# ariana-spalter/human-robot-gym

Measured on AMD Instinct MI355X. Metric: env steps/sec (whole node), ReachHuman+shield 4096 envs, higher is better.
Workload: dtype f64

## Files before the change

human-robot-gym_amd/_lib.py:

```python
import ctypes
import os
import subprocess

from ._cstruct import CONST, EnvState, BoxState, StackState, HammerState, ModelDesc, ClipTable

_HERE = os.path.dirname(os.path.abspath(__file__))
LIB_PATH = os.path.join(_HERE, "libhrgym_hip.so")
_variant = None
SRC = os.path.join(_HERE, "csrc", "hrgym_hip.hip")
SRC_BOX = os.path.join(_HERE, "csrc", "hrgym_box.hip")
SRC_HO = os.path.join(_HERE, "csrc", "hrgym_handover.hip")
SRC_LIFT = os.path.join(_HERE, "csrc", "hrgym_lift.hip")
SRC_STACK = os.path.join(_HERE, "csrc", "hrgym_stack.hip")
SRC_HAMMER = os.path.join(_HERE, "csrc", "hrgym_hammer.hip")
SRC_HULLS = os.path.join(_HERE, "csrc", "hrgym_hulls.hip")
SRC_BOX_HULLS = os.path.join(_HERE, "csrc", "hrgym_box_hulls.hip")

EXPORTS = [
    "hrg_last_error", "hrg_version", "hrg_state_bytes", "hrg_batch_create", "hrg_batch_destroy", "hrg_batch_reset",
    "hrg_batch_step", "hrg_batch_contacts", "hrg_batch_capsules", "hrg_batch_get_state", "hrg_batch_set_state",
    "hrg_batch_kernel_time", "hrg_batch_enable_taps", "hrg_box_bytes", "hrg_batch_get_box", "hrg_batch_set_box", "hrg_batch_get_states", "hrg_batch_set_states",
    "hrg_batch_check_actions", "hrg_stack_bytes", "hrg_batch_get_stack", "hrg_batch_set_stack", "hrg_batch_launch_order",
    "hrg_hammer_bytes", "hrg_batch_get_hammer", "hrg_batch_set_hammer", "hrg_test_hull_queries",
    "hrg_test_hull_box_queries", "hrg_batch_mpr_fallbacks",
]


def build_library(force=False, verbose=False):
    deps = [SRC, SRC_BOX, SRC_HO, SRC_LIFT, SRC_STACK, SRC_HAMMER, SRC_HULLS, SRC_BOX_HULLS] + [os.path.join(_HERE, "csrc", f) for f in ("hrgym_device.h", "hrgym_kernels.h", "hrgym_hull.h")] + [
        os.path.join(os.path.dirname(_HERE), "include", f) for f in ("hrgym.h", "hrgym_state.h")]
    if not force and os.path.exists(LIB_PATH) and all(os.path.getmtime(LIB_PATH) >= os.path.getmtime(d) for d in deps):
        return LIB_PATH
    cmd = ["hipcc", "--offload-arch=gfx950", "-O3", "-std=c++17", "-shared", "-fPIC", "-Wno-unused-value", "-Xarch_device", "-fapprox-func", "-mllvm", "-disable-machine-licm", "-o", LIB_PATH,
           SRC, SRC_BOX, SRC_HO, SRC_LIFT, SRC_STACK, SRC_HAMMER, SRC_HULLS, SRC_BOX_HULLS]
    if verbose:
        print(" ".join(cmd))
    subprocess.check_call(cmd)
    return LIB_PATH


_lib = None


def use_variant_library(path):
    global _variant
    if _lib is not None:
        raise RuntimeError("use_variant_library() must be called before the library is loaded")
    _variant = os.path.abspath(path)


def variant_library():
    return _variant


def load_library():
    global _lib
    if _lib is not None:
# ... 1 lines not shown
    for var in ("HRG_LIB_PATH", "HRG_PHASE_MASK"):
        if os.environ.get(var):
            raise RuntimeError(f"{var} is set: the library no longer honours it (use _lib.use_variant_library() / a -DHRG_STAMPS diagnostic build); unset it")
    path = _variant or LIB_PATH
    if not os.path.exists(path):
        raise RuntimeError(f"{path} is missing: run `python -c 'import __graft_entry__ as g; g.build()'` (hipcc --offload-arch=gfx950). "
                           "There is no CPU fallback for the stepper.")
    lib = ctypes.CDLL(path)
    vp, i32, i64 = ctypes.c_void_p, ctypes.c_int32, ctypes.c_int64
    lib.hrg_last_error.restype = ctypes.c_char_p
    lib.hrg_version.restype = ctypes.c_char_p
    lib.hrg_state_bytes.restype = ctypes.c_size_t
    lib.hrg_batch_create.argtypes = [ctypes.POINTER(ModelDesc), ctypes.POINTER(ClipTable), i32, i64, i32, ctypes.POINTER(vp)]
    lib.hrg_batch_destroy.argtypes = [vp]
    lib.hrg_batch_destroy.restype = None
    lib.hrg_batch_reset.argtypes = [vp, vp, vp, vp]
    lib.hrg_batch_step.argtypes = [vp] * 8
    lib.hrg_batch_contacts.argtypes = [vp, vp, vp]
    lib.hrg_batch_launch_order.argtypes = [vp, vp, vp]
    lib.hrg_batch_capsules.argtypes = [vp, vp, vp, vp]
    lib.hrg_batch_get_state.argtypes = [vp, i32, vp, ctypes.c_size_t]
    lib.hrg_batch_set_state.argtypes = [vp, i32, vp, ctypes.c_size_t]
    lib.hrg_batch_get_states.argtypes = [vp, vp, i32, vp, vp]
    lib.hrg_batch_set_states.argtypes = [vp, vp, i32, vp, vp]
    lib.hrg_box_bytes.restype = ctypes.c_size_t
    lib.hrg_batch_get_box.argtypes = [vp, i32, vp, ctypes.c_size_t]
    lib.hrg_batch_set_box.argtypes = [vp, i32, vp, ctypes.c_size_t]
    lib.hrg_hammer_bytes.restype = ctypes.c_size_t
    lib.hrg_batch_get_hammer.argtypes = [vp, i32, vp, ctypes.c_size_t]
    lib.hrg_batch_set_hammer.argtypes = [vp, i32, vp, ctypes.c_size_t]
    lib.hrg_test_hull_queries.argtypes = [vp, vp, vp, i32, vp]
    lib.hrg_test_hull_box_queries.argtypes = [vp, vp, vp, i32, vp]
    lib.hrg_batch_mpr_fallbacks.argtypes = [vp, ctypes.POINTER(i64)]
    lib.hrg_stack_bytes.restype = ctypes.c_size_t
    lib.hrg_batch_get_stack.argtypes = [vp, i32, vp, ctypes.c_size_t]
    lib.hrg_batch_set_stack.argtypes = [vp, i32, vp, ctypes.c_size_t]
    lib.hrg_batch_enable_taps.argtypes = [vp, i32]
    lib.hrg_batch_check_actions.argtypes = [vp, vp, vp, vp]
    lib.hrg_batch_kernel_time.argtypes = [vp, ctypes.POINTER(ctypes.c_double), ctypes.POINTER(i64)]
    if lib.hrg_state_bytes() != ctypes.sizeof(EnvState):
        raise RuntimeError("hrg_env_state layout mismatch between header mirror and library: rebuild")
    _lib = lib
    return lib


class HrgError(RuntimeError):
    pass


def _check(lib, rc):
    if rc != 0:
        raise HrgError(f"hrgym error {rc}: {lib.hrg_last_error().decode()}")


class HipBatch:

    def __init__(self, desc, clips, n_envs, env_id0=0, device=0, out=None):
        import torch
        if not torch.cuda.is_available():
            raise RuntimeError("HipBatch needs a ROCm GPU (torch.cuda.is_available() is False); there is no CPU fallback")
        self.torch = torch
        self.lib = load_library()
        self.n = int(n_envs)
        self.device = torch.device("cuda", device)
        self._clips = clips
        table = clips.table()
# ... 104 lines not shown
        _check(self.lib, self.lib.hrg_batch_get_hammer(self.h, int(e), ctypes.byref(s), ctypes.sizeof(s)))
        return s

    def set_hammer(self, e, s):
        _check(self.lib, self.lib.hrg_batch_set_hammer(self.h, int(e), ctypes.byref(s), ctypes.sizeof(s)))

    def get_stack(self, e):
        s = StackState()
        _check(self.lib, self.lib.hrg_batch_get_stack(self.h, int(e), ctypes.byref(s), ctypes.sizeof(s)))
        return s

    def set_stack(self, e, s):
        _check(self.lib, self.lib.hrg_batch_set_stack(self.h, int(e), ctypes.byref(s), ctypes.sizeof(s)))

    def contacts(self):
        import numpy as np
        pairs = np.zeros((self.n, CONST["HRG_NCON_MAX"], 2), np.int32)
        ncon = np.zeros(self.n, np.int32)
        _check(self.lib, self.lib.hrg_batch_contacts(self.h, pairs.ctypes.data_as(ctypes.c_void_p), ncon.ctypes.data_as(ctypes.c_void_p)))
        return pairs, ncon

    def launch_order(self):
        import numpy as np
        order = np.zeros(self.n, np.int32)
        nb = ctypes.c_int32(0)
        _check(self.lib, self.lib.hrg_batch_launch_order(self.h, order.ctypes.data_as(ctypes.c_void_p), ctypes.byref(nb)))
        return order, int(nb.value)

    def mpr_fallbacks(self):
        c = ctypes.c_int64()
        _check(self.lib, self.lib.hrg_batch_mpr_fallbacks(self.h, ctypes.byref(c)))
        return c.value

    def enable_taps(self, on=True):
        _check(self.lib, self.lib.hrg_batch_enable_taps(self.h, int(bool(on))))

    def capsules(self):
        import numpy as np
        r = np.zeros((self.n, CONST["HRG_NSHIELD_RCAP"], 7))
        h = np.zeros((self.n, CONST["HRG_NHCAP_MAX"], 7))
        nh = np.zeros(self.n, np.int32)
        vp = ctypes.c_void_p
        _check(self.lib, self.lib.hrg_batch_capsules(self.h, r.ctypes.data_as(vp), h.ctypes.data_as(vp), nh.ctypes.data_as(vp)))
        return r, h, nh

    def kernel_time(self):
        ms, n = ctypes.c_double(), ctypes.c_int64()
        _check(self.lib, self.lib.hrg_batch_kernel_time(self.h, ctypes.byref(ms), ctypes.byref(n)))
        return ms.value, n.value

    def close(self):
        if getattr(self, "h", None) and self.h.value:
            self.lib.hrg_batch_destroy(self.h)
            self.h = ctypes.c_void_p()

    def __del__(self):
        try:
            self.close()
        except Exception:
            pass
```

human-robot-gym_amd/csrc/hrgym_device.h:

```cpp
#pragma once
#include <hip/hip_runtime.h>
#include <stdint.h>

#include "../../include/hrgym.h"
#include "../../include/hrgym_state.h"

#define NV HRG_NV
#define NARM HRG_NARM
#ifndef HRG_BOX
#define HRG_BOX 0
#endif
#ifndef HRG_LIFT
#define HRG_LIFT 0
#endif
#ifndef HRG_HANDOVER
#define HRG_HANDOVER 0
#endif
#ifndef HRG_STACK
#define HRG_STACK 0
#endif
#ifndef HRG_HULLS
#define HRG_HULLS 0
#endif
#ifndef HRG_HAMMER
#define HRG_HAMMER 0
#endif
#define HRG_BASE_TU (!HRG_BOX && !HRG_STACK && !HRG_HAMMER && !HRG_HULLS)
#define NVT HRG_NVT
#if HRG_HAMMER
#define NVS HRG_NV_HAMMER
#define NCON_DYN HRG_NCON_DYN_HAMMER
#define HM_OB NV
#define HM_ON (NV + 6)
#define HM_OH (NV + 8)
#elif HRG_STACK
#define NVS HRG_NV_STACK
#define NCON_DYN HRG_NCON_DYN_STACK
#define NCUBE HRG_NCUBE
#elif HRG_BOX
#define NVS NVT
#define NCON_DYN HRG_NCON_DYN_BOX
#else
#define NVS NV
#define NCON_DYN HRG_NCON_DYN
#endif
#define BODY_BOX 100
#define DI __device__ __forceinline__
#ifndef HRG_MIN_WAVES
#define HRG_MIN_WAVES 4
#endif
#ifndef HRG_PHASE
#define HRG_PHASE __device__ __forceinline__
#endif
#define PH_DYNTERMS HRG_PHASE
#define PH_HUMAN HRG_PHASE
#define PH_SHIELD HRG_PHASE
#define PH_COLLIDE HRG_PHASE
#define PH_CLASSIFY HRG_PHASE
#define PH_DYNSTEP HRG_PHASE
#define HRG_PI 3.14159265358979323846
// ... 20 lines not shown
#define STAMP_FLUSH(lane)
#define COUNT(k, n) do { if (threadIdx.x == 0) g_acc[k] += (n); } while (0)
#define STAMP_FINAL(lane) do { __syncthreads(); if ((lane) < 32) atomicAdd(&g_stamps[lane], g_acc[lane]); { unsigned long long _te; STAMP_NOW(_te); if (_te - g_tbeg > g_slow_thresh) { if ((lane) < 32) atomicAdd(&g_stamps_slow[lane], g_acc[lane]); if ((lane) == 32) atomicAdd(&g_stamps_slow[32], 1ull); if ((lane) == 33) atomicAdd(&g_stamps_slow[33], _te - g_tbeg); } } if ((lane) < 32 && blockIdx.x < 16384) g_envacc[blockIdx.x][lane] = g_acc[lane]; if ((lane) == 0 && blockIdx.x < 16384) { unsigned long long _t; STAMP_NOW(_t); g_envcyc[blockIdx.x][0] = g_tbeg; g_envcyc[blockIdx.x][1] = _t; unsigned _hw, _xcc; asm volatile("s_getreg_b32 %0, hwreg(HW_REG_HW_ID)\n\ts_getreg_b32 %1, hwreg(HW_REG_XCC_ID)" : "=s"(_hw), "=s"(_xcc)); g_envcyc[blockIdx.x][2] = ((unsigned long long)_xcc << 32) | _hw; } } while (0)
#else
#define STAMP_DECL
#define STAMP_INIT(lane)
#define STAMP(k)
#define STAMP_FLUSH(lane)
#define COUNT(k, n)
#define STAMP_FINAL(lane)
#endif

struct DevModel {
  hrg_model_desc m;
  double Rbase[9];
  double Rq[NV][9];
  int32_t anc_mask[NV];
  int32_t hb_maxdepth;
  double sol_K, sol_Bd;
  double rcap_hl[HRG_NRCAP], hcap_hl[HRG_NHB];
  int32_t hb_njump;
  int32_t hb_jump[4][HRG_NHB];
  int32_t phase_mask;
  hrg_path brake_full;
  double brake_T, brake_ds;
  int32_t hc_n;
  int32_t hc_kind[HRG_NHCAP_MAX], hc_j1[HRG_NHCAP_MAX], hc_j2[HRG_NHCAP_MAX];
  double hc_th[HRG_NHCAP_MAX], hc_v[HRG_NHCAP_MAX], hc_a[HRG_NHCAP_MAX], hc_len[HRG_NHCAP_MAX];
  int32_t n_self;
  int32_t self_i[64], self_j[64];
  int32_t n_chk;
  int32_t chk_i[32], chk_j[32];
  hrg_clip_table clips;
  const double* hull_dev;
  double hull_cen[HRG_NHULL][3];
  unsigned long long* mpr_fallback;
};

static inline void hull_centroids(const double* verts, const int32_t* off, double cen[HRG_NHULL][3]) {
  for (int h = 0; h < HRG_NHULL; h++) {
    double s[3] = {0, 0, 0};
    for (int i = off[h]; i < off[h + 1]; i++) for (int a = 0; a < 3; a++) s[a] += verts[3 * i + a];
    for (int a = 0; a < 3; a++) cen[h][a] = s[a] / (double)(off[h + 1] - off[h]);
  }
}

struct Contact {
  int32_t g1, g2, b1, b2;
  double dist, n[3], pos[3];
};

#define ROW_CON0 24
#define ROW_WELD0 (ROW_CON0 + 4 * NCON_DYN)
#if HRG_HAMMER
#define HROW_NFRIC 8
#define HROW_LIM0 9
#define HROW_NLIM 25
#define HROW_EQ0 27
#define HROW_CON0 36
#define HROW_NEQ 9
#define NROW 128
#elif HRG_STACK
#define SROW_WELD0 24
#define SROW_CON0 36
#define NROW HRG_NROW_STACK
#elif HRG_BOX && (HRG_HANDOVER || HRG_LIFT)
// ... 730 lines not shown
```

human-robot-gym_amd/csrc/hrgym_hip.hip:

```cpp
#include <hip/hip_runtime.h>

#include <cmath>
#include <cstdio>
#include <cstring>
#include <cstdlib>
#include <memory>
#include <string>
#include <vector>

#include "hrgym_kernels.h"

template <class MD>
DI void impedance(const MD& m, double x0, double* imp) {
  const double d0 = m.solimp[0], dmax = m.solimp[1], width = m.solimp[2], mid = m.solimp[3], power = m.solimp[4];
  const double x = fabs(x0) / width;
  double y;
  if (x >= 1) y = 1;
  else if (x <= 0) y = 0;
  else if (x <= mid) { const double u = x / mid; y = u * u * mid; }
  else { const double u = (1 - x) / (1 - mid); y = 1 - u * u * (1 - mid); }
  (void)power;
  *imp = d0 + y * (dmax - d0);
}

// ... 2820 lines not shown
  const double* src = (const double*)(states + e);
  double* dst = (double*)&L.st;
  constexpr int NW = (int)(sizeof(hrg_env_state) / sizeof(double));
  for (int k = lane; k < NW; k += 64) dst[k] = src[k];
  wave_sync();
  env_reset(dm, lane, env_id0 + e, obs ? obs + (size_t)e * HRG_OBS_DIM : nullptr);
  wave_sync();
  hrg_env_state* st_out = states;
  asm volatile("" : "+s"(st_out));
  double* out = (double*)(st_out + e);
  for (int k = lane; k < NW; k += 64) out[k] = dst[k];
#if HRG_BOX || HRG_STACK || HRG_HAMMER
  box_store(boxes, e, lane);
#endif
}

#if HRG_BASE_TU
__global__ __launch_bounds__(64 * HRG_WG_WAVES, HRG_KERNEL_WAVES) void hrg_check_kernel(const DevModel* __restrict__ dm_, const hrg_env_state* __restrict__ states, const double* __restrict__ actions,
                                                                          uint8_t* __restrict__ collides, int n_envs) {
  const int e = hrg_env(), lane = hrg_lane();
  if (e >= n_envs) return;
  Lds& L = g_L;
  const double* src = (const double*)(states + e);
  double* dst = (double*)&L.st;
  constexpr int NW = (int)(sizeof(hrg_env_state) / sizeof(double));
  for (int k = lane; k < NW; k += 64) dst[k] = src[k];
  if (lane < NV) L.act[lane] = lane < HRG_ACT_DIM ? actions[(size_t)e * HRG_ACT_DIM + lane] : 0.0;
  wave_sync();
  const ModelPtr dm = uniform_model(dm_);
  action_goal(dm, lane, L.act);
  const bool hit = config_collides(dm_, lane);
  if (lane == 0) collides[e] = hit ? 1 : 0;
}
#endif

extern "C" __attribute__((visibility("hidden"))) void hrg_box_launch_step(int n_envs, hipStream_t st, const DevModel* dm, hrg_env_state* states, double* actions, float* obs, float* term_obs,
                                                                           float* reward, uint8_t* done, int32_t* info, double* dbg_r, double* dbg_h, int32_t* dbg_nh, int64_t env_id0,
                                                                           float* scratch_obs, hrg_box_state* boxes, StepOrder ord);
extern "C" __attribute__((visibility("hidden"))) void hrg_box_launch_reset(int n_envs, hipStream_t st, const DevModel* dm, hrg_env_state* states, const uint8_t* mask, float* obs,
                                                                            int64_t env_id0, hrg_box_state* boxes);
#if HRG_BASE_TU
extern "C" __attribute__((visibility("hidden"))) void hrg_stack_launch_step(int n_envs, hipStream_t st, const DevModel* dm, hrg_env_state* states, double* actions, float* obs, float* term_obs,
                                                                             float* reward, uint8_t* done, int32_t* info, double* dbg_r, double* dbg_h, int32_t* dbg_nh, int64_t env_id0,
                                                                             float* scratch_obs, hrg_stack_state* stacks, StepOrder ord);
extern "C" __attribute__((visibility("hidden"))) void hrg_stack_launch_reset(int n_envs, hipStream_t st, const DevModel* dm, hrg_env_state* states, const uint8_t* mask, float* obs,
                                                                              int64_t env_id0, hrg_stack_state* stacks);
#endif
#if HRG_BASE_TU
extern "C" __attribute__((visibility("hidden"))) void hrg_hammer_launch_step(int n_envs, hipStream_t st, const DevModel* dm, hrg_env_state* states, double* actions, float* obs, float* term_obs,
                                                                              float* reward, uint8_t* done, int32_t* info, double* dbg_r, double* dbg_h, int32_t* dbg_nh, int64_t env_id0,
                                                                              float* scratch_obs, hrg_hammer_state* hammers, StepOrder ord);
extern "C" __attribute__((visibility("hidden"))) void hrg_hammer_launch_reset(int n_envs, hipStream_t st, const DevModel* dm, hrg_env_state* states, const uint8_t* mask, float* obs,
                                                                               int64_t env_id0, hrg_hammer_state* hammers);
extern "C" __attribute__((visibility("hidden"))) void hrg_ho_launch_step(int n_envs, hipStream_t st, const DevModel* dm, hrg_env_state* states, double* actions, float* obs, float* term_obs,
                                                                          float* reward, uint8_t* done, int32_t* info, double* dbg_r, double* dbg_h, int32_t* dbg_nh, int64_t env_id0,
                                                                          float* scratch_obs, hrg_box_state* boxes, StepOrder ord);
extern "C" __attribute__((visibility("hidden"))) void hrg_ho_launch_reset(int n_envs, hipStream_t st, const DevModel* dm, hrg_env_state* states, const uint8_t* mask, float* obs,
                                                                           int64_t env_id0, hrg_box_state* boxes);
extern "C" __attribute__((visibility("hidden"))) void hrg_lift_launch_step(int n_envs, hipStream_t st, const DevModel* dm, hrg_env_state* states, double* actions, float* obs, float* term_obs,
                                                                            float* reward, uint8_t* done, int32_t* info, double* dbg_r, double* dbg_h, int32_t* dbg_nh, int64_t env_id0,
                                                                            float* scratch_obs, hrg_box_state* boxes, StepOrder ord);
extern "C" __attribute__((visibility("hidden"))) void hrg_lift_launch_reset(int n_envs, hipStream_t st, const DevModel* dm, hrg_env_state* states, const uint8_t* mask, float* obs,
                                                                             int64_t env_id0, hrg_box_state* boxes);
#endif
#if HRG_BASE_TU
extern "C" __attribute__((visibility("hidden"))) void hrg_box_hull_launch_step(int n_envs, hipStream_t st, const DevModel* dm, hrg_env_state* states, double* actions, float* obs, float* term_obs,
// ... 91 lines not shown
#define hrg_debug_envcyc hrg_debug_envcyc_ho
#elif HRG_LIFT
#define hrg_debug_envacc hrg_debug_envacc_lift
#define hrg_debug_envcyc hrg_debug_envcyc_lift
#elif HRG_BOX
#define hrg_debug_envacc hrg_debug_envacc_box
#define hrg_debug_envcyc hrg_debug_envcyc_box
#elif HRG_HULLS
#define hrg_debug_envacc hrg_debug_envacc_hull
#define hrg_debug_envcyc hrg_debug_envcyc_hull
#endif
#if 1
extern "C" int hrg_debug_envacc(unsigned long long* out, int n) { return hipMemcpyFromSymbol(out, HIP_SYMBOL(g_envacc), sizeof(unsigned long long) * 32 * n) == hipSuccess ? 0 : -1; }
extern "C" int hrg_debug_envcyc(unsigned long long* out, int n) { return hipMemcpyFromSymbol(out, HIP_SYMBOL(g_envcyc), sizeof(unsigned long long) * 3 * n) == hipSuccess ? 0 : -1; }
#endif
#endif

#if HRG_BASE_TU

static thread_local std::string g_err;
static int fail(int code, const std::string& msg) { g_err = msg; return code; }
#define HIPCHK(x)                                                                                         \
  do {                                                                                                    \
    hipError_t _e = (x);                                                                                  \
    if (_e != hipSuccess) return fail(HRG_ERR_HIP, std::string(#x) + ": " + hipGetErrorString(_e));        \
  } while (0)

struct hrg_batch {
  int device = 0;
  int32_t n_envs = 0;
  int64_t env_id0 = 0;
  DevModel* d_model = nullptr;
  double* d_frames = nullptr;
  double* d_hull = nullptr;
  bool hulls = false;
  unsigned long long* d_mpr_fallback = nullptr;
  hrg_env_state* d_states = nullptr;
  double* d_rcaps = nullptr;
  double* d_hcaps = nullptr;
  int32_t* d_nh = nullptr;
  float* d_scratch_obs = nullptr;
  hrg_box_state* d_boxes = nullptr;
  hrg_stack_state* d_stacks = nullptr;
  hrg_hammer_state* d_hammers = nullptr;
  int32_t* d_order = nullptr;
  int32_t parity = 0;
  int32_t task = HRG_TASK_REACH;
  bool timing = false;
  bool taps = false;
  std::vector<std::pair<hipEvent_t, hipEvent_t>> events;
  std::vector<std::pair<hipEvent_t, hipEvent_t>> pool;
};

static int32_t* fair_table(int device) {
  static int32_t* tab[64] = {nullptr};
  if (device < 0 || device >= 64) return nullptr;
  if (!tab[device]) {
    int32_t* p = nullptr;
    if (hipMalloc(&p, sizeof(int32_t) * HRG_FAIR_SLOTS) != hipSuccess) return nullptr;
    if (hipMemset(p, 0, sizeof(int32_t) * HRG_FAIR_SLOTS) != hipSuccess) { hipFree(p); return nullptr; }
    tab[device] = p;
  }
  return tab[device];
}

static void mat_from_quat(double* M, const double* q) {
  double w = q[0], x = q[1], y = q[2], z = q[3];
  M[0] = 1 - 2 * (y * y + z * z); M[1] = 2 * (x * y - w * z); M[2] = 2 * (x * z + w * y);
  M[3] = 2 * (x * y + w * z); M[4] = 1 - 2 * (x * x + z * z); M[5] = 2 * (y * z - w * x);
  M[6] = 2 * (x * z - w * y); M[7] = 2 * (y * z + w * x); M[8] = 1 - 2 * (x * x + y * y);
}

extern "C" {

const char* hrg_last_error(void) { return g_err.c_str(); }
const char* hrg_version(void) { return "hrgym-hip 0.1.0 (gfx950)"; }
size_t hrg_state_bytes(void) { return sizeof(hrg_env_state); }
size_t hrg_box_bytes(void) { return sizeof(hrg_box_state); }
size_t hrg_stack_bytes(void) { return sizeof(hrg_stack_state); }
size_t hrg_hammer_bytes(void) { return sizeof(hrg_hammer_state); }

int hrg_batch_create(const hrg_model_desc* desc, const hrg_clip_table* clips, int32_t n_envs, int64_t env_id0, int32_t device, hrg_batch** out) {
  if (!desc || !clips || !out || n_envs <= 0) return fail(HRG_ERR_INVALID, "null argument or n_envs <= 0");
  if (desc->failsafe_sdot != 0.0) return fail(HRG_ERR_INVALID, "failsafe_sdot must be 0: SSM / OFF brake to a stop, PFL computes its speed from pfl_v_safe / pfl_reach");
  if (desc->shield_type == HRG_SHIELD_PFL) {
    if (!(desc->pfl_v_safe > 0)) return fail(HRG_ERR_INVALID, "PFL: pfl_v_safe must be positive");
    for (int j = 0; j < NARM; j++) if (!(desc->pfl_reach[j] > 0)) return fail(HRG_ERR_INVALID, "PFL: pfl_reach must be positive");
  }
  for (int i = 0; i < NARM; i++)
    if (!(desc->jnt_damping[i] >= 0 && desc->timestep * desc->jnt_damping[i] * desc->dof_invweight0[i] < 1e-3))
      return fail(HRG_ERR_UNSUPPORTED, "arm joint damping too large for the implicit-damping expansion (h d / M must stay below 1e-3; robot.xml: 1e-4)");
  if ((desc->jnt_damping[NARM] > 0) != (desc->jnt_damping[NARM + 1] > 0)) return fail(HRG_ERR_UNSUPPORTED, "the two finger slides must both carry damping, or neither");
  if (desc->solimp[4] != 2.0) return fail(HRG_ERR_UNSUPPORTED, "solimp power must be 2 (MuJoCo's default): the HIP stepper evaluates the impedance sigmoid as a square");
  if (clips->n_clips < 1 || clips->n_clips > HRG_MAX_CLIPS || clips->n_clips != desc->n_clips) return fail(HRG_ERR_INVALID, "clip table / desc.n_clips mismatch");
  for (int i = 0; i < NV; i++) {
    if ((i < NARM) != (desc->jnt_type[i] == 0)) return fail(HRG_ERR_INVALID, "expected 6 hinges followed by 2 slides");
    if (i < NARM && desc->body_parent[i] != i - 1) return fail(HRG_ERR_INVALID, "arm must be a serial chain");
// ... 96 lines not shown
  hm->hc_n = n;
  int ns = 0;
  for (int i = 0; i < HRG_NRCAP; i++)
    for (int j = i + 1; j < HRG_NRCAP; j++)
      if ((desc->rcap_selfmask[i] >> j) & 1u) { hm->self_i[ns] = i; hm->self_j[ns] = j; ns++; }
  hm->n_self = ns;
  int nc = 0;
  for (int i = 0; i < 8; i++)
    for (int j = i + 1; j < 8; j++)
      if (((desc->chk_selfmask[i] >> j) & 1u) && nc < 32) { hm->chk_i[nc] = i; hm->chk_j[nc] = j; nc++; }
  hm->n_chk = nc;
  hm->phase_mask = 0xff;
  {
    double se, ve, ae;
    path_plan(&hm->brake_full, 0.0, 1.0, 0.0, desc->failsafe_sdot, desc->path_amax, desc->path_jmax);
    hm->brake_T = path_total(&hm->brake_full);
    path_eval(&hm->brake_full, hm->brake_T, desc->failsafe_sdot, &se, &ve, &ae);
    hm->brake_ds = se;
  }
#ifdef HRG_STAMPS
  if (const char* pm = getenv("HRG_PHASE_MASK")) hm->phase_mask = atoi(pm);
#endif
  const size_t fbytes = sizeof(double) * HRG_FRAME_DIM * (size_t)clips->total_frames;
  int64_t tot = 0;
  for (int c = 0; c < clips->n_clips; c++) {
    if (clips->clip_len[c] < 1 || clips->clip_offset[c] != tot) { return bail(HRG_ERR_INVALID, "clip table must be densely packed"); }
    tot += clips->clip_len[c];
  }
  if (tot != clips->total_frames) { return bail(HRG_ERR_INVALID, "clip table total_frames mismatch"); }
  HIPCHK_C(hipMalloc(&b->d_frames, fbytes));
  HIPCHK_C(hipMemcpy(b->d_frames, clips->frames, fbytes, hipMemcpyHostToDevice));
  hm->clips = *clips;
  hm->clips.frames = b->d_frames;
  hm->hull_dev = nullptr;
  if (desc->robot_hulls) {
    if (!(desc->task == HRG_TASK_REACH || desc->task == HRG_TASK_PICK_PLACE || desc->task == HRG_TASK_INSPECTION || desc->task == HRG_TASK_POINTING || desc->task == HRG_TASK_REACH_BOX))
      return bail(HRG_ERR_UNSUPPORTED, "robot_hulls: the hull variants of the step kernel exist for ReachHuman and the cube tasks (PickPlace, Inspection, ReachHuman with reach_box)");
    b->hulls = true;
    if (!desc->hull_verts || desc->hull_off[0] != 0) return bail(HRG_ERR_INVALID, "robot_hulls: hull_verts / hull_off missing");
    for (int h = 0; h < HRG_NHULL; h++)
      if (!(desc->hull_off[h + 1] > desc->hull_off[h] + 3 && desc->hull_off[h + 1] <= 1000000)) return bail(HRG_ERR_INVALID, "robot_hulls: every hull needs at least four vertices");
    const size_t hbytes = sizeof(double) * 3 * (size_t)desc->hull_off[HRG_NHULL];
    HIPCHK_C(hipMalloc(&b->d_hull, hbytes));
    HIPCHK_C(hipMemcpy(b->d_hull, desc->hull_verts, hbytes, hipMemcpyHostToDevice));
    hm->hull_dev = b->d_hull;
    hull_centroids(desc->hull_verts, desc->hull_off, hm->hull_cen);
    HIPCHK_C(hipMalloc(&b->d_mpr_fallback, sizeof(unsigned long long)));
    HIPCHK_C(hipMemset(b->d_mpr_fallback, 0, sizeof(unsigned long long)));
    hm->mpr_fallback = b->d_mpr_fallback;
  }
  HIPCHK_C(hipMalloc(&b->d_model, sizeof(DevModel)));
  HIPCHK_C(hipMemcpy(b->d_model, hm, sizeof(DevModel), hipMemcpyHostToDevice));
  HIPCHK_C(hipMalloc(&b->d_states, sizeof(hrg_env_state) * (size_t)n_envs));
  std::vector<hrg_env_state> init((size_t)n_envs);
  memset(init.data(), 0, sizeof(hrg_env_state) * (size_t)n_envs);
  for (auto& s : init) s.episode = -1;
  HIPCHK_C(hipMemcpy(b->d_states, init.data(), sizeof(hrg_env_state) * (size_t)n_envs, hipMemcpyHostToDevice));
  HIPCHK_C(hipMalloc(&b->d_rcaps, sizeof(double) * 7 * HRG_NSHIELD_RCAP * (size_t)n_envs));
  HIPCHK_C(hipMalloc(&b->d_hcaps, sizeof(double) * 7 * HRG_NHCAP_MAX * (size_t)n_envs));
  HIPCHK_C(hipMalloc(&b->d_nh, sizeof(int32_t) * (size_t)n_envs));
  HIPCHK_C(hipMalloc(&b->d_scratch_obs, sizeof(float) * HRG_OBS_DIM * (size_t)n_envs));
  HIPCHK_C(hipMemset(b->d_rcaps, 0, sizeof(double) * 7 * HRG_NSHIELD_RCAP * (size_t)n_envs));
  HIPCHK_C(hipMemset(b->d_hcaps, 0, sizeof(double) * 7 * HRG_NHCAP_MAX * (size_t)n_envs));
  HIPCHK_C(hipMemset(b->d_nh, 0, sizeof(int32_t) * (size_t)n_envs));
  HIPCHK_C(hipMalloc(&b->d_boxes, sizeof(hrg_box_state) * (size_t)n_envs));
  HIPCHK_C(hipMemset(b->d_boxes, 0, sizeof(hrg_box_state) * (size_t)n_envs));
  if (desc->task == HRG_TASK_HAMMERING) {
    HIPCHK_C(hipMalloc(&b->d_hammers, sizeof(hrg_hammer_state) * (size_t)n_envs));
    HIPCHK_C(hipMemset(b->d_hammers, 0, sizeof(hrg_hammer_state) * (size_t)n_envs));
  }
  if (desc->task == HRG_TASK_STACKING) {
    HIPCHK_C(hipMalloc(&b->d_stacks, sizeof(hrg_stack_state) * (size_t)n_envs));
    HIPCHK_C(hipMemset(b->d_stacks, 0, sizeof(hrg_stack_state) * (size_t)n_envs));
  }
  {
    std::vector<int32_t> ord(2 * (size_t)n_envs + 4, 0);
    for (int32_t e = 0; e < n_envs; e++) ord[e] = ord[(size_t)n_envs + e] = e;
    HIPCHK_C(hipMalloc(&b->d_order, sizeof(int32_t) * ord.size()));
    HIPCHK_C(hipMemcpy(b->d_order, ord.data(), sizeof(int32_t) * ord.size(), hipMemcpyHostToDevice));
  }
#undef HIPCHK_C
  *out = b;
  return HRG_OK;
}

void hrg_batch_destroy(hrg_batch* b) {
  if (!b) return;
  hipSetDevice(b->device);
  hipDeviceSynchronize();
  for (auto& p : b->events) { hipEventDestroy(p.first); hipEventDestroy(p.second); }
  for (auto& p : b->pool) { hipEventDestroy(p.first); hipEventDestroy(p.second); }
  hipFree(b->d_model); hipFree(b->d_frames); hipFree(b->d_hull); hipFree(b->d_mpr_fallback); hipFree(b->d_states); hipFree(b->d_rcaps); hipFree(b->d_hcaps); hipFree(b->d_nh); hipFree(b->d_scratch_obs); hipFree(b->d_boxes); hipFree(b->d_stacks); hipFree(b->d_hammers); hipFree(b->d_order);
  delete b;
}

int hrg_batch_reset(hrg_batch* b, const uint8_t* mask_dev, float* obs_dev, void* stream) {
  if (!b) return fail(HRG_ERR_INVALID, "null batch");
  HIPCHK(hipSetDevice(b->device));
  if (b->task == HRG_TASK_HAMMERING) hrg_hammer_launch_reset(b->n_envs, (hipStream_t)stream, b->d_model, b->d_states, mask_dev, obs_dev, b->env_id0, b->d_hammers);
  else if (b->task == HRG_TASK_STACKING) hrg_stack_launch_reset(b->n_envs, (hipStream_t)stream, b->d_model, b->d_states, mask_dev, obs_dev, b->env_id0, b->d_stacks);
  else if (b->task == HRG_TASK_LIFTING) hrg_lift_launch_reset(b->n_envs, (hipStream_t)stream, b->d_model, b->d_states, mask_dev, obs_dev, b->env_id0, b->d_boxes);
  else if (HRG_IS_HANDOVER(b->task)) hrg_ho_launch_reset(b->n_envs, (hipStream_t)stream, b->d_model, b->d_states, mask_dev, obs_dev, b->env_id0, b->d_boxes);
  else if (b->task != HRG_TASK_REACH && b->hulls) hrg_box_hull_launch_reset(b->n_envs, (hipStream_t)stream, b->d_model, b->d_states, mask_dev, obs_dev, b->env_id0, b->d_boxes);
  else if (b->task != HRG_TASK_REACH) hrg_box_launch_reset(b->n_envs, (hipStream_t)stream, b->d_model, b->d_states, mask_dev, obs_dev, b->env_id0, b->d_boxes);
  else if (b->hulls) hrg_hull_launch_reset(b->n_envs, (hipStream_t)stream, b->d_model, b->d_states, mask_dev, obs_dev, b->env_id0);
  else hipLaunchKernelGGL(hrg_reset_kernel, HRG_LAUNCH_DIMS(b->n_envs), 0, (hipStream_t)stream, b->d_model, b->d_states, mask_dev, obs_dev, b->env_id0, b->d_boxes, b->n_envs);
  HIPCHK(hipGetLastError());
  return HRG_OK;
}

int hrg_batch_check_actions(hrg_batch* b, const double* actions_dev, uint8_t* collides_dev, void* stream) {
  if (!b || !actions_dev || !collides_dev) return fail(HRG_ERR_INVALID, "null argument");
  HIPCHK(hipSetDevice(b->device));
  hipLaunchKernelGGL(hrg_check_kernel, HRG_LAUNCH_DIMS(b->n_envs), 0, (hipStream_t)stream, b->d_model, b->d_states, actions_dev, collides_dev, b->n_envs);
  HIPCHK(hipGetLastError());
  return HRG_OK;
}

int hrg_batch_step(hrg_batch* b, double* actions_dev, float* obs_dev, float* term_obs_dev, float* reward_dev, uint8_t* done_dev, int32_t* info_dev, void* stream) {
  if (!b || !actions_dev || !obs_dev || !reward_dev || !done_dev || !info_dev) return fail(HRG_ERR_INVALID, "null argument");
  HIPCHK(hipSetDevice(b->device));
  hipStream_t st = (hipStream_t)stream;
  std::pair<hipEvent_t, hipEvent_t> ev;
  if (b->timing) {
    if (!b->pool.empty()) { ev = b->pool.back(); b->pool.pop_back(); }
    else { HIPCHK(hipEventCreate(&ev.first)); HIPCHK(hipEventCreate(&ev.second)); }
// ... 205 lines not shown
```

human-robot-gym_amd/csrc/hrgym_kernels.h:

```cpp
#pragma once
#include "hrgym_device.h"
#if HRG_HULLS
#include "hrgym_hull.h"
#endif

DI void robot_chain_fk(const DevModel* __restrict__ dm_, int lane, bool shield_on) {
  const ModelPtr dm = uniform_model(dm_);
  Lds& L = g_L;
  double* sc = &L.rc[0][0];
  if (lane < 3 * NARM && (lane >= 2 * NARM || shield_on)) {
    const int cfg = lane / NARM, i = lane - NARM * cfg;
    const double q = cfg == 0 ? L.cq[i] : (cfg == 1 ? L.qe[i] : L.st.qpos[i]);
    double sn, cs;
    sincos_small(q, &sn, &cs);
    sc[2 * lane] = sn; sc[2 * lane + 1] = cs;
  }
  wave_sync();
  if (lane < 9 && (lane >= 6 || shield_on)) {
    const auto& m = dm->m;
    const int cfg = lane / 3, row = lane - 3 * cfg;
    double r0 = dm->Rbase[3 * row], r1 = dm->Rbase[3 * row + 1], r2 = dm->Rbase[3 * row + 2];
    double p = m.base_pos[row];
#pragma unroll 1
    for (int i = 0; i < NARM; i++) {
// ... 239 lines not shown
      const int hd = lane == bl ? 0 : 1;
      const double sn = hd == 0 ? -1.0 : 1.0;
      double Rm[9], q[4], site[3], t[3];
      for (int a = 0; a < 3; a++) { Rm[3 * a] = -sn * R[3 * a + 2]; Rm[3 * a + 1] = R[3 * a + 1]; Rm[3 * a + 2] = sn * R[3 * a]; }
      const double tr = Rm[0] + Rm[4] + Rm[8];
      if (tr > 0) { const double S = fsqrt(tr + 1.0) * 2; q[0] = 0.25 * S; q[1] = (Rm[7] - Rm[5]) / S; q[2] = (Rm[2] - Rm[6]) / S; q[3] = (Rm[3] - Rm[1]) / S; }
      else if (Rm[0] > Rm[4] && Rm[0] > Rm[8]) { const double S = fsqrt(1.0 + Rm[0] - Rm[4] - Rm[8]) * 2; q[0] = (Rm[7] - Rm[5]) / S; q[1] = 0.25 * S; q[2] = (Rm[1] + Rm[3]) / S; q[3] = (Rm[2] + Rm[6]) / S; }
      else if (Rm[4] > Rm[8]) { const double S = fsqrt(1.0 + Rm[4] - Rm[0] - Rm[8]) * 2; q[0] = (Rm[2] - Rm[6]) / S; q[1] = (Rm[1] + Rm[3]) / S; q[2] = 0.25 * S; q[3] = (Rm[5] + Rm[7]) / S; }
      else { const double S = fsqrt(1.0 + Rm[8] - Rm[0] - Rm[4]) * 2; q[0] = (Rm[3] - Rm[1]) / S; q[1] = (Rm[2] + Rm[6]) / S; q[2] = (Rm[5] + Rm[7]) / S; q[3] = 0.25 * S; }
      m3mulv(t, R, m.hb_anchor[b]);
      v3add(site, p, t);
      for (int a = 0; a < 4; a++) L.hm.mocap_quat[hd][a] = q[a];
      for (int a = 0; a < 3; a++) L.hm.mocap_pos[hd][a] = site[a];
    }
  }
#endif
  {
    const int k = lane < HRG_NHJ ? lane : 0;
    const int sb = m.meas_body[k];
    double Rs[9], ps[3];
#pragma unroll
    for (int a = 0; a < 9; a++) Rs[a] = __shfl(R[a], sb, 64);
#pragma unroll
    for (int a = 0; a < 3; a++) ps[a] = __shfl(p[a], sb, 64);
    if (lane < HRG_NHJ) {
      double t[3];
      m3mulv(t, Rs, m.hb_anchor[sb]);
      v3add(L.st.human_site[k], ps, t);
    }
  }
  wave_sync();
}

DI void human_pose_fk(const DevModel* __restrict__ dm_, int lane, int clip, int at, int hold_body = -1, int hold_left = 0) {
  const ModelPtr dm = uniform_model(dm_);
  Lds& L = g_L;
  const auto& m = dm->m;
  hrg_env_state& s = L.st;
  const double* fr = dm->clips.frames + (dm->clips.clip_offset[clip] + at) * HRG_FRAME_DIM;
  double qi[4] = {dm->clips.clip_quat[clip][3], dm->clips.clip_quat[clip][0], dm->clips.clip_quat[clip][1], dm->clips.clip_quat[clip][2]};
  double qbi[4], Rbi[9], pa[3], pr[3], mp[3], mq[4], q1[4];
  quatmul(qbi, m.human_base_quat, qi);
  quat2mat(Rbi, qbi);
  for (int a = 0; a < 3; a++) pa[a] = fr[a] + dm->clips.clip_pos_offset[clip][a];
  m3mulv(pr, Rbi, pa);
  v3add(mp, pr, s.human_pos_offset);
  double qa[4] = {fr[6], fr[3], fr[4], fr[5]};
  quatmul(q1, s.human_rot_offset, qbi);
  quatmul(mq, q1, qa);
  human_fk_lanes(dm_, lane, mp, mq, fr + 7, hold_body, hold_left);
}

#if HRG_BOX || HRG_STACK || HRG_HAMMER
DI double loop_prop(ModelPtr dm, int64_t gid, int episode, int ai, int clip, int k, int speed) {
  double base = speed ? dm->clips.clip_loop_speed[clip][k % HRG_MAX_LOOP] : dm->clips.clip_loop_amp[clip][k % HRG_MAX_LOOP];
  if (k >= HRG_MAX_LOOP) base = speed ? dm->clips.clip_loop2_speed[clip][k - HRG_MAX_LOOP] : dm->clips.clip_loop2_amp[clip][k - HRG_MAX_LOOP];
  const double sf = speed ? dm->clips.clip_loop_speed_std[clip] : dm->clips.clip_loop_amp_std[clip];
  const double z = clampd(rng_gauss(dm->m.seed, (uint64_t)gid, (uint64_t)episode, STREAM_LOOP, (uint64_t)((ai * 2 * HRG_MAX_LOOP + k) * 2 + speed)), -3.0, 3.0);
  return base * exp(z * log(sf));
}
DI double layered_sines(ModelPtr dm, int64_t gid, int episode, int ai, int clip, int kfirst, int n, double t, double start) {
  static_assert(2 * HRG_MAX_LOOP <= 64, "one lane per loop property");
  const int lane = hrg_lane(), kk = lane % HRG_MAX_LOOP, sp = (lane / HRG_MAX_LOOP) & 1;
  const double mine = loop_prop(dm, gid, episode, ai, clip, kfirst + (kk < n ? kk : 0), sp);
  double sum = 0;
  for (int k = 0; k < n; k++) {
    const double A = __shfl(mine, k), S = __shfl(mine, HRG_MAX_LOOP + k);
    sum += A * sin((t - start) / (A / S)) + start;
  }
  return sum - start * (double)(n - 1);
}
#endif

PH_HUMAN void human_control(const DevModel* __restrict__ dm_, int lane, int64_t gid) {
  const ModelPtr dm = uniform_model(dm_);
  Lds& L = g_L;
  const auto& m = dm->m;
  hrg_env_state& s = L.st;
  int control_time = (int)floor((double)s.low_level_time / m.anim_step_length);
  int at = control_time - s.anim_start_time;
  int anim_index = s.anim_index, anim_start = s.anim_start_time;
  int clip = clip_of(dm, gid, s.episode, anim_index);
#if HRG_BOX
// ... 1194 lines not shown
```

include/hrgym.h:

```cpp
#ifndef HRGYM_H
#define HRGYM_H

#include <stddef.h>
#include <stdint.h>

#ifdef __cplusplus
extern "C" {
#endif

#define HRG_NARM 6
#define HRG_NFINGER 2
#define HRG_NV (HRG_NARM + HRG_NFINGER)
#define HRG_NHB 24
#define HRG_NHJ 23
#define HRG_NHQ 69
#define HRG_NRCAP 10
#define HRG_NHULL 7
#define HRG_NSHIELD_RCAP 7
#define HRG_NBODYPART_MAX 20
#define HRG_NEXTREMITY_MAX 4
#define HRG_NHCAP_MAX 64
#define HRG_LTT_NSEG 12
#define HRG_OBS_DIM 64
#define HRG_ACT_DIM 7
// ... 250 lines not shown
const char* hrg_version(void);

size_t hrg_state_bytes(void);

int hrg_batch_create(const hrg_model_desc* desc, const hrg_clip_table* clips, int32_t n_envs,
                     int64_t env_id0, int32_t device, hrg_batch** out);
void hrg_batch_destroy(hrg_batch* b);

int hrg_batch_reset(hrg_batch* b, const uint8_t* mask_dev, float* obs_dev, void* stream);

int hrg_batch_step(hrg_batch* b, double* actions_dev, float* obs_dev, float* term_obs_dev,
                   float* reward_dev, uint8_t* done_dev, int32_t* info_dev, void* stream);

int hrg_batch_contacts(hrg_batch* b, int32_t* pairs_host, int32_t* ncon_host);
int hrg_batch_capsules(hrg_batch* b, double* robot_host, double* human_host, int32_t* n_human_host);
int hrg_batch_launch_order(hrg_batch* b, int32_t* order_host, int32_t* n_busy_host);
int hrg_batch_enable_taps(hrg_batch* b, int32_t on);
int hrg_batch_get_state(hrg_batch* b, int32_t env, void* buf_host, size_t bytes);
int hrg_batch_set_state(hrg_batch* b, int32_t env, const void* buf_host, size_t bytes);
int hrg_batch_get_states(hrg_batch* b, const int32_t* envs_host, int32_t n, void* states_host, void* boxes_host);
int hrg_batch_set_states(hrg_batch* b, const int32_t* envs_host, int32_t n, const void* states_host, const void* boxes_host);
size_t hrg_box_bytes(void);
int hrg_batch_get_box(hrg_batch* b, int32_t env, void* buf_host, size_t bytes);
int hrg_batch_set_box(hrg_batch* b, int32_t env, const void* buf_host, size_t bytes);
size_t hrg_stack_bytes(void);
int hrg_batch_get_stack(hrg_batch* b, int32_t env, void* buf_host, size_t bytes);
int hrg_batch_set_stack(hrg_batch* b, int32_t env, const void* buf_host, size_t bytes);
size_t hrg_hammer_bytes(void);
int hrg_batch_get_hammer(hrg_batch* b, int32_t env, void* buf_host, size_t bytes);
int hrg_batch_set_hammer(hrg_batch* b, int32_t env, const void* buf_host, size_t bytes);
int hrg_test_hull_queries(const double* verts_host, const int32_t* off_host, const void* queries_host, int32_t n, double* out_host);
int hrg_test_hull_box_queries(const double* verts_host, const int32_t* off_host, const void* queries_host, int32_t n, double* out_host);
int hrg_batch_mpr_fallbacks(hrg_batch* b, int64_t* count_host);

int hrg_batch_check_actions(hrg_batch* b, const double* actions_dev, uint8_t* collides_dev, void* hip_stream);

int hrg_batch_kernel_time(hrg_batch* b, double* avg_ms, int64_t* n_launches);

#ifdef __cplusplus
}
#endif
#endif
```

Before: 4.076 million.

## Precompute per-frame human pose table at batch creation for reach and lift

At batch creation, a kernel runs the human forward kinematics once for every clip frame in a root-relative frame and stores the capsule endpoints, joint sites and root position in a device table. During stepping, reach and lift tasks then rebuild the human pose with one rotation plus translation per lane from the table, replacing the per-step tree FK. The cost is extra device memory and an init-time kernel. Hold-body handling is dropped on this path, and a debug comparison kernel is added to check the table against live FK.

Result: faster. 4.500 million, median of 6 (+10.4%).

```diff
diff --git a/human-robot-gym_amd/_lib.py b/human-robot-gym_amd/_lib.py
--- a/human-robot-gym_amd/_lib.py
+++ b/human-robot-gym_amd/_lib.py
@@ -22,7 +22,7 @@
     "hrg_batch_kernel_time", "hrg_batch_enable_taps", "hrg_box_bytes", "hrg_batch_get_box", "hrg_batch_set_box", "hrg_batch_get_states", "hrg_batch_set_states",
     "hrg_batch_check_actions", "hrg_stack_bytes", "hrg_batch_get_stack", "hrg_batch_set_stack", "hrg_batch_launch_order",
     "hrg_hammer_bytes", "hrg_batch_get_hammer", "hrg_batch_set_hammer", "hrg_test_hull_queries",
-    "hrg_test_hull_box_queries", "hrg_batch_mpr_fallbacks",
+    "hrg_test_hull_box_queries", "hrg_batch_mpr_fallbacks", "hrg_batch_pose_table_bytes", "hrg_debug_pose_compare",
 ]
 
 
@@ -90,6 +90,8 @@
     lib.hrg_test_hull_queries.argtypes = [vp, vp, vp, i32, vp]
     lib.hrg_test_hull_box_queries.argtypes = [vp, vp, vp, i32, vp]
     lib.hrg_batch_mpr_fallbacks.argtypes = [vp, ctypes.POINTER(i64)]
+    lib.hrg_batch_pose_table_bytes.argtypes = [vp, ctypes.POINTER(i64)]
+    lib.hrg_debug_pose_compare.argtypes = [vp, vp, i32, vp]
     lib.hrg_stack_bytes.restype = ctypes.c_size_t
     lib.hrg_batch_get_stack.argtypes = [vp, i32, vp, ctypes.c_size_t]
     lib.hrg_batch_set_stack.argtypes = [vp, i32, vp, ctypes.c_size_t]
@@ -260,6 +262,11 @@
         _check(self.lib, self.lib.hrg_batch_mpr_fallbacks(self.h, ctypes.byref(c)))
         return c.value
 
+    def pose_table_bytes(self):
+        c = ctypes.c_int64()
+        _check(self.lib, self.lib.hrg_batch_pose_table_bytes(self.h, ctypes.byref(c)))
+        return c.value
+
     def enable_taps(self, on=True):
         _check(self.lib, self.lib.hrg_batch_enable_taps(self.h, int(bool(on))))
 
diff --git a/human-robot-gym_amd/csrc/hrgym_device.h b/human-robot-gym_amd/csrc/hrgym_device.h
--- a/human-robot-gym_amd/csrc/hrgym_device.h
+++ b/human-robot-gym_amd/csrc/hrgym_device.h
@@ -26,6 +26,11 @@
 #define HRG_HAMMER 0
 #endif
 #define HRG_BASE_TU (!HRG_BOX && !HRG_STACK && !HRG_HAMMER && !HRG_HULLS)
+#define HRG_POSE_TABLE ((!HRG_BOX && !HRG_STACK && !HRG_HAMMER) || HRG_LIFT)
+#define HRG_POSE_HCAP 0
+#define HRG_POSE_SITE (6 * HRG_NHB)
+#define HRG_POSE_ROOT (HRG_POSE_SITE + 3 * HRG_NHJ)
+#define HRG_POSE_DIM (HRG_POSE_ROOT + 3)
 #define NVT HRG_NVT
 #if HRG_HAMMER
 #define NVS HRG_NV_HAMMER
@@ -112,6 +117,7 @@
   int32_t n_chk;
   int32_t chk_i[32], chk_j[32];
   hrg_clip_table clips;
+  const double* pose_tab;
   const double* hull_dev;
   double hull_cen[HRG_NHULL][3];
   unsigned long long* mpr_fallback;
diff --git a/human-robot-gym_amd/csrc/hrgym_hip.hip b/human-robot-gym_amd/csrc/hrgym_hip.hip
--- a/human-robot-gym_amd/csrc/hrgym_hip.hip
+++ b/human-robot-gym_amd/csrc/hrgym_hip.hip
@@ -2876,6 +2876,56 @@
   const bool hit = config_collides(dm_, lane);
   if (lane == 0) collides[e] = hit ? 1 : 0;
 }
+
+__global__ __launch_bounds__(64) void hrg_pose_table_kernel(const DevModel* __restrict__ dm_, double* __restrict__ tab) {
+  const ModelPtr dm = uniform_model(dm_);
+  const int lane = hrg_lane();
+  const int64_t f = (int64_t)blockIdx.x;
+  if (f >= dm->clips.total_frames) return;
+  Lds& L = g_L;
+  int clip = 0;
+  for (int c = 1; c < dm->clips.n_clips; c++)
+    if (f >= dm->clips.clip_offset[c]) clip = c;
+  const double* fr = dm->clips.frames + f * HRG_FRAME_DIM;
+  double qbi[4], qa[4], c[3], mq[4];
+  human_root(dm, clip, fr, c, qbi, qa);
+  quatmul(mq, qbi, qa);
+  const double p0[3] = {0, 0, 0};
+  human_fk_lanes(dm_, lane, p0, mq, fr + 7);
+  double* e = tab + f * HRG_POSE_DIM;
+  for (int k = lane; k < 6 * HRG_NHB; k += 64) e[HRG_POSE_HCAP + k] = (&L.hcap[0][0])[k];
+  for (int k = lane; k < 3 * HRG_NHJ; k += 64) e[HRG_POSE_SITE + k] = (&L.st.human_site[0][0])[k];
+  if (lane < 3) e[HRG_POSE_ROOT + lane] = c[lane];
+}
+
+struct PoseQuery { double pos_off[3], rot_off[4]; int32_t clip, at; };
+__global__ __launch_bounds__(64) void hrg_pose_compare_kernel(const DevModel* __restrict__ dm_, const PoseQuery* __restrict__ q, int n, double* __restrict__ out) {
+  const ModelPtr dm = uniform_model(dm_);
+  const int lane = hrg_lane(), k = (int)blockIdx.x;
+  if (k >= n) return;
+  Lds& L = g_L;
+  hrg_env_state& s = L.st;
+  if (lane < 3) s.human_pos_offset[lane] = q[k].pos_off[lane];
+  if (lane < 4) s.human_rot_offset[lane] = q[k].rot_off[lane];
+  wave_sync();
+  const int clip = __builtin_amdgcn_readfirstlane(q[k].clip), at = __builtin_amdgcn_readfirstlane(q[k].at);
+  const int64_t f = dm->clips.clip_offset[clip] + at;
+  const double* fr = dm->clips.frames + f * HRG_FRAME_DIM;
+  double qbi[4], qa[4], c[3], mp[3], mq[4], q1[4];
+  human_root(dm, clip, fr, c, qbi, qa);
+  v3add(mp, c, s.human_pos_offset);
+  quatmul(q1, s.human_rot_offset, qbi);
+  quatmul(mq, q1, qa);
+  human_fk_lanes(dm_, lane, mp, mq, fr + 7);
+  constexpr int NP = 6 * HRG_NHB + 3 * HRG_NHJ;
+  double* o = out + (size_t)k * 2 * NP;
+  for (int j = lane; j < 6 * HRG_NHB; j += 64) o[j] = (&L.hcap[0][0])[j];
+  for (int j = lane; j < 3 * HRG_NHJ; j += 64) o[6 * HRG_NHB + j] = (&s.human_site[0][0])[j];
+  wave_sync();
+  human_pose_from_table(dm, lane, f);
+  for (int j = lane; j < 6 * HRG_NHB; j += 64) o[NP + j] = (&L.hcap[0][0])[j];
+  for (int j = lane; j < 3 * HRG_NHJ; j += 64) o[NP + 6 * HRG_NHB + j] = (&s.human_site[0][0])[j];
+}
 #endif
 
 extern "C" __attribute__((visibility("hidden"))) void hrg_box_launch_step(int n_envs, hipStream_t st, const DevModel* dm, hrg_env_state* states, double* actions, float* obs, float* term_obs,
@@ -3033,6 +3083,8 @@
   int64_t env_id0 = 0;
   DevModel* d_model = nullptr;
   double* d_frames = nullptr;
+  double* d_pose = nullptr;
+  size_t pose_bytes = 0;
   double* d_hull = nullptr;
   bool hulls = false;
   unsigned long long* d_mpr_fallback = nullptr;
@@ -3064,6 +3116,8 @@
   }
   return tab[device];
 }
+
+static bool hrg_task_uses_pose_table(int task) { return task == HRG_TASK_REACH || task == HRG_TASK_LIFTING; }
 
 static void mat_from_quat(double* M, const double* q) {
   double w = q[0], x = q[1], y = q[2], z = q[3];
@@ -3226,6 +3280,12 @@
   HIPCHK_C(hipMemcpy(b->d_frames, clips->frames, fbytes, hipMemcpyHostToDevice));
   hm->clips = *clips;
   hm->clips.frames = b->d_frames;
+  hm->pose_tab = nullptr;
+  if (hrg_task_uses_pose_table(desc->task)) {
+    b->pose_bytes = sizeof(double) * HRG_POSE_DIM * (size_t)clips->total_frames;
+    HIPCHK_C(hipMalloc(&b->d_pose, b->pose_bytes));
+    hm->pose_tab = b->d_pose;
+  }
   hm->hull_dev = nullptr;
   if (desc->robot_hulls) {
     if (!(desc->task == HRG_TASK_REACH || desc->task == HRG_TASK_PICK_PLACE || desc->task == HRG_TASK_INSPECTION || desc->task == HRG_TASK_POINTING || desc->task == HRG_TASK_REACH_BOX))
@@ -3245,6 +3305,11 @@
   }
   HIPCHK_C(hipMalloc(&b->d_model, sizeof(DevModel)));
   HIPCHK_C(hipMemcpy(b->d_model, hm, sizeof(DevModel), hipMemcpyHostToDevice));
+  if (b->d_pose) {
+    hipLaunchKernelGGL(hrg_pose_table_kernel, dim3((unsigned)clips->total_frames), dim3(64), 0, 0, b->d_model, b->d_pose);
+    HIPCHK_C(hipGetLastError());
+    HIPCHK_C(hipDeviceSynchronize());
+  }
   HIPCHK_C(hipMalloc(&b->d_states, sizeof(hrg_env_state) * (size_t)n_envs));
   std::vector<hrg_env_state> init((size_t)n_envs);
   memset(init.data(), 0, sizeof(hrg_env_state) * (size_t)n_envs);
@@ -3284,8 +3349,36 @@
   hipDeviceSynchronize();
   for (auto& p : b->events) { hipEventDestroy(p.first); hipEventDestroy(p.second); }
   for (auto& p : b->pool) { hipEventDestroy(p.first); hipEventDestroy(p.second); }
-  hipFree(b->d_model); hipFree(b->d_frames); hipFree(b->d_hull); hipFree(b->d_mpr_fallback); hipFree(b->d_states); hipFree(b->d_rcaps); hipFree(b->d_hcaps); hipFree(b->d_nh); hipFree(b->d_scratch_obs); hipFree(b->d_boxes); hipFree(b->d_stacks); hipFree(b->d_hammers); hipFree(b->d_order);
+  hipFree(b->d_model); hipFree(b->d_frames); hipFree(b->d_pose); hipFree(b->d_hull); hipFree(b->d_mpr_fallback); hipFree(b->d_states); hipFree(b->d_rcaps); hipFree(b->d_hcaps); hipFree(b->d_nh); hipFree(b->d_scratch_obs); hipFree(b->d_boxes); hipFree(b->d_stacks); hipFree(b->d_hammers); hipFree(b->d_order);
   delete b;
+}
+
+int hrg_batch_pose_table_bytes(hrg_batch* b, int64_t* bytes_host) {
+  if (!b || !bytes_host) return fail(HRG_ERR_INVALID, "null argument");
+  *bytes_host = (int64_t)b->pose_bytes;
+  return HRG_OK;
+}
+
+int hrg_debug_pose_compare(hrg_batch* b, const void* queries_host, int32_t n, double* out_host) {
+  if (!b || !queries_host || !out_host || n <= 0) return fail(HRG_ERR_INVALID, "null argument or n <= 0");
+  if (!b->d_pose) return fail(HRG_ERR_UNSUPPORTED, "this batch's task keeps the live tree kinematics (no pose table)");
+  DevModel hm;
+  HIPCHK(hipSetDevice(b->device));
+  HIPCHK(hipMemcpy(&hm, b->d_model, sizeof hm, hipMemcpyDeviceToHost));
+  const PoseQuery* qh = (const PoseQuery*)queries_host;
+  for (int k = 0; k < n; k++)
+    if (qh[k].clip < 0 || qh[k].clip >= hm.clips.n_clips || qh[k].at < 0 || qh[k].at >= hm.clips.clip_len[qh[k].clip]) return fail(HRG_ERR_INVALID, "query outside the clip set");
+  const size_t ob = sizeof(double) * 2 * (6 * HRG_NHB + 3 * HRG_NHJ) * (size_t)n;
+  PoseQuery* dq = nullptr;
+  double* dout = nullptr;
+  bool ok = false;
+  if (hipMalloc(&dq, sizeof(PoseQuery) * (size_t)n) == hipSuccess && hipMalloc(&dout, ob) == hipSuccess &&
+      hipMemcpy(dq, qh, sizeof(PoseQuery) * (size_t)n, hipMemcpyHostToDevice) == hipSuccess) {
+    hipLaunchKernelGGL(hrg_pose_compare_kernel, dim3((unsigned)n), dim3(64), 0, 0, b->d_model, dq, (int)n, dout);
+    ok = hipDeviceSynchronize() == hipSuccess && hipMemcpy(out_host, dout, ob, hipMemcpyDeviceToHost) == hipSuccess;
+  }
+  hipFree(dq); hipFree(dout);
+  return ok ? HRG_OK : fail(HRG_ERR_HIP, "hrg_debug_pose_compare: device allocation / copy / launch failed");
 }
 
 int hrg_batch_reset(hrg_batch* b, const uint8_t* mask_dev, float* obs_dev, void* stream) {
diff --git a/human-robot-gym_amd/csrc/hrgym_kernels.h b/human-robot-gym_amd/csrc/hrgym_kernels.h
--- a/human-robot-gym_amd/csrc/hrgym_kernels.h
+++ b/human-robot-gym_amd/csrc/hrgym_kernels.h
@@ -295,23 +295,59 @@
   wave_sync();
 }
 
+DI void human_root(ModelPtr dm, int clip, const double* fr, double* c, double* qbi, double* qa) {
+  const double qi[4] = {dm->clips.clip_quat[clip][3], dm->clips.clip_quat[clip][0], dm->clips.clip_quat[clip][1], dm->clips.clip_quat[clip][2]};
+  double Rbi[9], pa[3];
+  quatmul(qbi, dm->m.human_base_quat, qi);
+  quat2mat(Rbi, qbi);
+  for (int a = 0; a < 3; a++) pa[a] = fr[a] + dm->clips.clip_pos_offset[clip][a];
+  m3mulv(c, Rbi, pa);
+  qa[0] = fr[6]; qa[1] = fr[3]; qa[2] = fr[4]; qa[3] = fr[5];
+}
+
+DI void human_pose_from_table(ModelPtr dm, int lane, int64_t f) {
+  Lds& L = g_L;
+  hrg_env_state& s = L.st;
+  const double* e = dm->pose_tab + f * HRG_POSE_DIM;
+  const bool cap = lane < HRG_NHB, site = !cap && lane < HRG_NHB + HRG_NHJ;
+  double y[6] = {0, 0, 0, 0, 0, 0};
+  if (cap) {
+    const double2* p = (const double2*)(e + HRG_POSE_HCAP + 6 * lane);
+    const double2 a = p[0], b = p[1], d = p[2];
+    y[0] = a.x; y[1] = a.y; y[2] = b.x; y[3] = b.y; y[4] = d.x; y[5] = d.y;
+  } else if (site) {
+    const double* p = e + HRG_POSE_SITE + 3 * (lane - HRG_NHB);
+    y[0] = p[0]; y[1] = p[1]; y[2] = p[2];
+  }
+  const double __attribute__((address_space(4)))* ec = (const double __attribute__((address_space(4)))*)(e + HRG_POSE_ROOT);
+  double R[9], o[3], x[3];
+  quat2mat(R, s.human_rot_offset);
+  v3add(o, s.human_pos_offset, ec);
+  m3mulv(x, R, y);
+  if (cap) {
+    v3add(&L.hcap[lane][0], o, x);
+    m3mulv(x, R, y + 3);
+    v3add(&L.hcap[lane][3], o, x);
+  } else if (site) v3add(L.st.human_site[lane - HRG_NHB], o, x);
+  wave_sync();
+}
+
 DI void human_pose_fk(const DevModel* __restrict__ dm_, int lane, int clip, int at, int hold_body = -1, int hold_left = 0) {
   const ModelPtr dm = uniform_model(dm_);
+#if HRG_POSE_TABLE
+  (void)hold_body; (void)hold_left;
+  human_pose_from_table(dm, lane, (int64_t)dm->clips.clip_offset[clip] + at);
+#else
   Lds& L = g_L;
-  const auto& m = dm->m;
   hrg_env_state& s = L.st;
   const double* fr = dm->clips.frames + (dm->clips.clip_offset[clip] + at) * HRG_FRAME_DIM;
-  double qi[4] = {dm->clips.clip_quat[clip][3], dm->clips.clip_quat[clip][0], dm->clips.clip_quat[clip][1], dm->clips.clip_quat[clip][2]};
-  double qbi[4], Rbi[9], pa[3], pr[3], mp[3], mq[4], q1[4];
-  quatmul(qbi, m.human_base_quat, qi);
-  quat2mat(Rbi, qbi);
-  for (int a = 0; a < 3; a++) pa[a] = fr[a] + dm->clips.clip_pos_offset[clip][a];
-  m3mulv(pr, Rbi, pa);
-  v3add(mp, pr, s.human_pos_offset);
-  double qa[4] = {fr[6], fr[3], fr[4], fr[5]};
+  double qbi[4], qa[4], c[3], mp[3], mq[4], q1[4];
+  human_root(dm, clip, fr, c, qbi, qa);
+  v3add(mp, c, s.human_pos_offset);
   quatmul(q1, s.human_rot_offset, qbi);
   quatmul(mq, q1, qa);
   human_fk_lanes(dm_, lane, mp, mq, fr + 7, hold_body, hold_left);
+#endif
 }
 
 #if HRG_BOX || HRG_STACK || HRG_HAMMER
diff --git a/include/hrgym.h b/include/hrgym.h
--- a/include/hrgym.h
+++ b/include/hrgym.h
@@ -306,6 +306,8 @@
 int hrg_test_hull_queries(const double* verts_host, const int32_t* off_host, const void* queries_host, int32_t n, double* out_host);
 int hrg_test_hull_box_queries(const double* verts_host, const int32_t* off_host, const void* queries_host, int32_t n, double* out_host);
 int hrg_batch_mpr_fallbacks(hrg_batch* b, int64_t* count_host);
+int hrg_batch_pose_table_bytes(hrg_batch* b, int64_t* bytes_host);
+int hrg_debug_pose_compare(hrg_batch* b, const void* queries_host, int32_t n, double* out_host);
 
 int hrg_batch_check_actions(hrg_batch* b, const double* actions_dev, uint8_t* collides_dev, void* hip_stream);
 
```
